# alexncoleman/WeaklySupervisedDL

Hardware: AMD Instinct MI355X
Metric: SegmentationModel train img/s at B=16 256x256 (higher is better)
Workload: dtype f32

## Files before the change

### weaklysuperviseddl_amd/csrc/conv_igemm.hip

```cpp
#include "common.h"

#include <type_traits>
#include <algorithm>
#include <cstdint>
#include <mutex>

typedef float f32x16 __attribute__((ext_vector_type(16)));

namespace {

constexpr int kThreads = 256;

struct ConvSrc {
    const float* x;
    const float* wt;
    const float* x_amax;
    int KH, KW, bh, ch, K, Cin;
    long long x_bs;
    unsigned x_bytes;
};

struct ConvP {
    const float* x;
    const float* wt;
    float* y;
    const float* scale;
    const float* shift;
    const float* res;
    int B, Cin, H, W, Cout, OH, OW, KH, KW;
    int ah, bh, ch, sh;
    int K;
    long long x_bs, y_bs, res_bs;
    int relu, accumulate;
    int P;
    unsigned x_bytes;
    int ksplit;
    float* slab;
    int ow0, own;
    int nb;
    int b_ow0[4], b_own[4], b_tile0[5];
    int grid_x;
    int xcd_py;
    int xcd_rowfast;
    int tile_img_major;
    const float* x_amax;
    float* y_amax;
    const uint8_t* acc_mask;
    const float* acc_base;
    int nsrc;
    ConvSrc src[3];
};

__device__ __forceinline__ float acc_prev(const ConvP& p, const float* ptr) {
    float o = *ptr;
    if (p.acc_mask) {
        const long long e = ptr - p.acc_base;
        if (!((p.acc_mask[e >> 3] >> (e & 7)) & 1)) o = 0.f;
    }
    return o;
}

template <int BM, int BN, int WM, bool ALIGNED>
__global__ __launch_bounds__(kThreads) void conv_igemm_kernel(ConvP p) {
    constexpr int BK = 16;
    constexpr int WN = 4 / WM;
    constexpr int MI = BM / WM / 32;
    constexpr int NI = BN / WN / 32;
    static_assert(MI >= 1 && NI >= 1 && MI * 32 * WM == BM && NI * 32 * WN == BN, "bad tile");
    constexpr int A_F4 = BK * BM / 4 / kThreads;
    constexpr int B_STEP = kThreads / BN;
    constexpr int B_PER = BK / B_STEP;

    __shared__ float As[2][BK * BM];
    __shared__ float Bs[2][BK * BN];
    __shared__ int vtaps[64];
    constexpr int kTab = ALIGNED ? 1 : 1024;
    __shared__ int ktab[kTab][2];

    const int tid = threadIdx.x;
    const int lane = tid & 63, wid = tid >> 6;
    const int wm = wid / WN, wn = wid % WN;
    const int m0 = blockIdx.y * BM;
    const int n0 = blockIdx.x * BN;
    const int OHOW = p.OH * p.OW;
    const int HW = p.H * p.W;
    const bool use_tab = !ALIGNED && p.K <= kTab;
    if (use_tab) {
        for (int k = tid; k < p.K; k += kThreads) {
            const int tp = k / p.Cin, ci = k - tp * p.Cin;
            const int ti = tp / p.KW, tj = tp - ti * p.KW;
            ktab[k][0] = ci * HW;
            ktab[k][1] = (int)(((unsigned)(ti * p.bh) << 16) | ((unsigned)(tj * p.bh) & 0xffffu));
        }
        __syncthreads();
    }

    const int pl = tid % BN, kr = tid / BN;
// ... 1103 lines not shown
            for (int pix = c0; pix < c0 + BK && pix < P && !any; ++pix) {
                const int r = pix % OHW, ih = (r / own) * stride + dh, iw = (ow0 + r % own) * stride + dw;
                any = ih >= 0 && ih < H && iw >= 0 && iw < W;
            }
            done += any;
            ++all;
        }
    }
    return all ? (double)done / (double)all : 1.0;
}

wsdl::Opt g_tile_threshold{400};
wsdl::Opt g_group_tps10{45};
constexpr int kNumCU = 256, kLdsPerCU = 160 * 1024;

template <int BM, int BN, int WM, int BK>
int launch_fast(const ConvP& p, hipStream_t s, dim3 grid) {
    grid.z = p.ksplit > 1 ? p.ksplit : 1;
    constexpr size_t static_lds = 2 * BK * (BM + BN) * sizeof(float) + 64 * sizeof(int);
    static std::once_flag once;
    std::call_once(once, [] {
        (void)hipFuncSetAttribute(reinterpret_cast<const void*>(&conv_igemm_fast_kernel<BM, BN, WM, BK>),
                                  hipFuncAttributeMaxDynamicSharedMemorySize, kLdsPerCU - (int)static_lds - 2048);
    });
    WSDL_TRACE("fp32_fast<%d,%d,%d> ks=%d nb=%d grid=%ux%ux%u", BM, BN, BK, p.ksplit, p.nb, grid.x, grid.y, grid.z);
    hipLaunchKernelGGL((conv_igemm_fast_kernel<BM, BN, WM, BK>), grid, dim3(kThreads), 0, s, p);
    WSDL_LAUNCH_CHECK();
    return WSDL_OK;
}

wsdl::Opt g_conv_split{1};
wsdl::Opt g_conv_arith{1};
bool split_eligible(int rows, int kc, int T) {
    return g_conv_split && kc % 16 == 0 && T <= 9 && split_layout_bytes(g_conv_arith, (long long)T * kc, rows) < (1ll << 31);
}

wsdl::Opt g_xcd_map{1};
int choose_xcd_py(const ConvP& p, int gx, int gy) {
    if (!g_xcd_map || p.ksplit > 1 || ((long long)gx * gy) % 8 != 0) return 0;
    const double wb = (g_conv_arith ? 4.0 : 6.0) * (double)p.K * p.Cout, xb = 4.0 * (double)p.B * p.Cin * p.H * p.W;
    int best = 0;
    double best_cost = 0.0;
    for (int py = 1; py <= 8; py *= 2) {
        const int px = 8 / py;
        if (gy % py || gx % px) continue;
        if (g_xcd_map > 10 && py != g_xcd_map - 10) continue;
        const double cost = wb * px + xb * py;
        if (!best || cost < best_cost) { best = py; best_cost = cost; }
    }
    if (g_xcd_map == 1 && (best <= 1 || best_cost > 0.9 * (wb * 8 + xb))) return 0;
    return best;
}

template <int BM, int BN, int WM, int BK>
int launch_split(const ConvP& p_in, hipStream_t s, dim3 grid) {
    ConvP p = p_in;
    grid.z = p.ksplit > 1 ? p.ksplit : 1;
    p.xcd_py = choose_xcd_py(p, grid.x, grid.y);
    p.tile_img_major = 0;
    constexpr bool MF = BK == 32;
    WSDL_TRACE("split<%d,%d,%d> ar=%d %s ks=%d xcd_py=%d nb=%d grid=%ux%ux%u", BM, BN, BK, (int)g_conv_arith,
               (MF && g_conv_arith) ? "mfma16x16x32" : "mfma32x32x16", p.ksplit, p.xcd_py, p.nb, grid.x, grid.y, grid.z);
    if (g_conv_arith == 2)
        hipLaunchKernelGGL((conv_igemm_split_kernel<BM, BN, WM, BK, kThreads, 2, MF>), grid, dim3(kThreads), 0, s, p);
    else if (g_conv_arith)
        hipLaunchKernelGGL((conv_igemm_split_kernel<BM, BN, WM, BK, kThreads, 1, MF>), grid, dim3(kThreads), 0, s, p);
    else
        hipLaunchKernelGGL((conv_igemm_split_kernel<BM, BN, WM, BK, kThreads, 0>), grid, dim3(kThreads), 0, s, p);
    WSDL_LAUNCH_CHECK();
    return WSDL_OK;
}

wsdl::Opt g_conv_il{1};
int launch_split_256x128(const ConvP& p_in, hipStream_t s) {
    ConvP p = p_in;
    dim3 grid(p.grid_x > 0 ? p.grid_x : wsdl::cdiv(p.P, 128), wsdl::cdiv(p.Cout, 256), p.ksplit > 1 ? p.ksplit : 1);
    p.xcd_py = choose_xcd_py(p, grid.x, grid.y);
    p.xcd_rowfast = 0;
    p.tile_img_major = 0;
    if (p.nsrc > 0 && grid.y % 2 == 0 && ((long long)grid.x * grid.y) % 8 == 0) {
        int py = 4;
        while (py > 1 && (grid.y % py || grid.x % (8 / py))) py /= 2;
        if (grid.y % py == 0 && grid.x % (8 / py) == 0) {
            p.xcd_py = py;
            p.xcd_rowfast = 1;
        }
    }
    WSDL_TRACE("split<256,128,16> ar=%d il=%d nsrc=%d ks=%d xcd_py=%d rowfast=%d imgmajor=%d nb=%d grid=%ux%ux%u", (int)g_conv_arith,
               (int)(g_conv_arith == 1 && g_conv_il), p.nsrc, p.ksplit, p.xcd_py, p.xcd_rowfast, p.tile_img_major, p.nb, grid.x, grid.y, grid.z);
    if (p.nsrc > 0) {
        if (g_conv_arith == 2) hipLaunchKernelGGL((conv_igemm_split_kernel<256, 128, 4, 16, 512, 2, false, true>), grid, dim3(512), 0, s, p);
        else if (g_conv_arith && g_conv_il)
            hipLaunchKernelGGL((conv_igemm_split_kernel<256, 128, 4, 16, 512, 1, false, true, true>), grid, dim3(512), 0, s, p);
        else if (g_conv_arith) hipLaunchKernelGGL((conv_igemm_split_kernel<256, 128, 4, 16, 512, 1, false, true>), grid, dim3(512), 0, s, p);
        else hipLaunchKernelGGL((conv_igemm_split_kernel<256, 128, 4, 16, 512, 0, false, true>), grid, dim3(512), 0, s, p);
        WSDL_LAUNCH_CHECK();
        return WSDL_OK;
    }
    if (g_conv_arith == 2) hipLaunchKernelGGL((conv_igemm_split_kernel<256, 128, 4, 16, 512, 2>), grid, dim3(512), 0, s, p);
    else if (g_conv_arith && g_conv_il)
        hipLaunchKernelGGL((conv_igemm_split_kernel<256, 128, 4, 16, 512, 1, false, false, true>), grid, dim3(512), 0, s, p);
    else if (g_conv_arith) hipLaunchKernelGGL((conv_igemm_split_kernel<256, 128, 4, 16, 512, 1>), grid, dim3(512), 0, s, p);
    else hipLaunchKernelGGL((conv_igemm_split_kernel<256, 128, 4, 16, 512, 0>), grid, dim3(512), 0, s, p);
    WSDL_LAUNCH_CHECK();
    return WSDL_OK;
}

template <int BM, int BN, int WM>
int launch_cfg(const ConvP& p, hipStream_t s, bool aligned, bool split) {
    dim3 grid(p.grid_x > 0 ? p.grid_x : wsdl::cdiv(p.P, BN), wsdl::cdiv(p.Cout, BM));
    constexpr bool kSmallTile = BM * BN <= 128 * 64;
    if (split) {
        if constexpr (kSmallTile) {
            if (p.Cin % 32 == 0) {
                return launch_split<BM, BN, WM, 32>(p, s, grid);
            }
        }
        return launch_split<BM, BN, WM, 16>(p, s, grid);
    } else if (aligned) {
        if constexpr (kSmallTile) {
            if (p.Cin % 32 == 0) {
                return launch_fast<BM, BN, WM, 32>(p, s, grid);
            }
        }
        return launch_fast<BM, BN, WM, 16>(p, s, grid);
    } else {
        WSDL_TRACE("fp32_generic<%d,%d> grid=%ux%u", BM, BN, grid.x, grid.y);
        hipLaunchKernelGGL((conv_igemm_kernel<BM, BN, WM, false>), grid, dim3(kThreads), 0, s, p);
    }
    WSDL_LAUNCH_CHECK();
    return WSDL_OK;
}

wsdl::Opt g_ksplit_target{512}, g_ksplit_max{8}, g_ksplit_min_chunks{4};
int igemm_ksplit(int P, int Cout, int Cin, int T, int dil) {
    if (Cin % 32 != 0 || Cout % 4 != 0 || Cout <= 64) return 1;
    const long long blocks = (long long)wsdl::cdiv(P, 64) * wsdl::cdiv(Cout, 128);
    const int nq = T * (Cin / 32);
    const long long b128 = (long long)wsdl::cdiv(P, 128) * wsdl::cdiv(Cout, 128);
    if (b128 >= 200 && b128 < g_tile_threshold && nq >= 64) return 2;
    if (blocks >= 160 || nq < 8) return 1;
    long long s = g_ksplit_target / blocks;
// ... 571 lines not shown
    WSDL_REQUIRE(ws_bytes >= wsdl_conv2d_fwd_group_workspace(n, k, dil, B, Cin, H, W, Cout) && (ws || ws_bytes == 0),
                 "conv2d_fwd_group: workspace too small");
    hipStream_t s = wsdl::as_stream(stream);
    ConvGroup grp{};
    grp.n = n;
    int order[4] = {0, 1, 2, 3};
    std::stable_sort(order, order + n, [&](int a, int b) {
        return group_max_taps(H, W, k[a], dil[a]) > group_max_taps(H, W, k[b], dil[b]); });
    unsigned char* wsp = static_cast<unsigned char*>(ws);
    int start = 0;
    double flops = 0.0, executed = 0.0, bytes = 4.0 * (double)B * Cin * H * W;
    const long long xbs = x_bs ? x_bs : (long long)Cin * H * W;
    for (int j = 0; j < n; ++j) {
        const int i = order[j];
        WSDL_REQUIRE(wt_fwd[i] && y[i], "conv2d_fwd_group: null problem %d", i);
        WSDL_REQUIRE((k[i] == 1 || k[i] == 3) && dil[i] >= 1, "conv2d_fwd_group: problem %d: 1x1 or 3x3, stride 1", i);
        WSDL_REQUIRE(split_eligible(Cout, Cin, k[i] * k[i]), "conv2d_fwd_group: problem %d is not on the split kernels", i);
        ConvP& p = grp.p[j];
        const int pad = dil[i] * (k[i] - 1) / 2;
        p.x = x; p.wt = static_cast<const float*>(wt_fwd[i]); p.y = y[i];
        p.B = B; p.Cin = Cin; p.H = H; p.W = W; p.Cout = Cout; p.OH = H; p.OW = W; p.KH = p.KW = k[i];
        p.ah = 1; p.bh = dil[i]; p.ch = -pad; p.sh = 1;
        p.K = k[i] * k[i] * Cin;
        p.x_bs = xbs;
        p.y_bs = (y_bs && y_bs[i]) ? y_bs[i] : (long long)Cout * H * W;
        p.res_bs = p.y_bs;
        WSDL_REQUIRE(p.x_bs >= (long long)Cin * H * W && p.y_bs >= (long long)Cout * H * W, "conv2d_fwd_group: batch stride smaller than an image");
        p.P = B * H * W;
        p.x_bytes = (unsigned)(((long long)(B - 1) * p.x_bs + (long long)Cin * H * W) * 4);
        p.x_amax = x_amax;
        p.ow0 = 0; p.own = W; p.nb = 1;
        Band bands[8];
        int nb = 1;
        bands[0] = Band{0, W};
        nb = column_bands(W, W, p.ah, p.bh, p.ch, p.sh, p.KW, bands);
        int tiles = 0;
        for (int b = 0; b < nb && nb > 1; ++b) {
            p.b_ow0[b] = bands[b].ow0;
            p.b_own[b] = bands[b].own;
            p.b_tile0[b] = tiles;
            tiles += wsdl::cdiv((long long)B * H * bands[b].own, 128);
        }
        p.nb = nb;
        p.b_tile0[nb > 1 ? nb : 0] = tiles;
        const int gx = nb > 1 ? tiles : wsdl::cdiv(p.P, 128), gy = Cout / 256;
        const int ks = group_ksplit(group_max_taps(H, W, k[i], dil[i]));
        p.ksplit = ks;
        if (ks > 1) {
            p.slab = reinterpret_cast<float*>(wsp);
            wsp += wsdl::align_up((size_t)ks * Cout * p.P * sizeof(float), 256);
        }
        p.xcd_py = (start % 8 == 0) ? choose_xcd_py(p, gx, gy) : 0;
        p.tile_img_major = k[i] > 1;
        grp.start[j] = start;
        grp.gx[j] = gx;
        grp.gy[j] = gy;
        start += gx * gy * ks;
        const double f = 2.0 * p.P * (double)Cout * p.K;
        flops += f;
        if (wsdl::prof_enabled()) {
            for (int b = 0; b < nb; ++b) {
                ConvP q = p;
                q.ow0 = bands[b].ow0; q.own = bands[b].own; q.P = B * H * q.own;
                executed += f * ((double)q.own / W) * igemm_executed_fraction(q, 128);
            }
        }
        bytes += 4.0 * ((double)p.K * Cout + (double)p.P * Cout);
    }
    grp.start[n] = start;
    {
        int ns = 0;
        bool same = true;
        for (int j = 0; j < n; ++j) {
            ns += grp.p[j].ksplit;
            same = same && grp.gx[j] * grp.gy[j] == grp.gx[0] * grp.gy[0];
        }
        if (same && ns <= 8 && (8 % ns == 0)) {
            grp.ns = ns;
            int s = 0;
            for (int j = 0; j < n; ++j)
                for (int z = 0; z < grp.p[j].ksplit; ++z) {
                    grp.s_prob[s] = j;
                    grp.s_slice[s] = z;
                    ++s;
                }
            for (int j = 0; j < n; ++j) grp.p[j].xcd_py = 0;
        }
    }
    {
        wsdl::ProfScope prof(WSDL_PROF_SPLIT_GROUP, s, flops, wsdl::prof_enabled() ? executed : flops, bytes);
        WSDL_TRACE("group split<256,128,16> ar=%d il=%d problems=%d streams=%d ks=%d/%d/%d/%d workgroups=%d", (int)g_conv_arith,
                   (int)(g_conv_arith == 1 && g_conv_il), n, grp.ns, grp.p[0].ksplit, n > 1 ? grp.p[1].ksplit : 0,
                   n > 2 ? grp.p[2].ksplit : 0, n > 3 ? grp.p[3].ksplit : 0, start);
        if (g_conv_arith == 2)
            hipLaunchKernelGGL((conv_igemm_split_group_kernel<256, 128, 4, 16, 512, 2>), dim3(start), dim3(512), 0, s, grp);
        else if (g_conv_arith && g_conv_il)
            hipLaunchKernelGGL((conv_igemm_split_group_kernel<256, 128, 4, 16, 512, 1, false, true>), dim3(start), dim3(512), 0, s, grp);
        else if (g_conv_arith)
            hipLaunchKernelGGL((conv_igemm_split_group_kernel<256, 128, 4, 16, 512, 1>), dim3(start), dim3(512), 0, s, grp);
        else
            hipLaunchKernelGGL((conv_igemm_split_group_kernel<256, 128, 4, 16, 512, 0>), dim3(start), dim3(512), 0, s, grp);
        WSDL_LAUNCH_CHECK();
    }
    for (int j = 0; j < n; ++j) {
        const ConvP& p = grp.p[j];
        if (p.ksplit <= 1) continue;
        const long long total = (long long)p.Cout * p.P;
        const bool vec4 = p.y_bs % 4 == 0 && (reinterpret_cast<uintptr_t>(p.y) & 15) == 0;
        if (vec4)
            hipLaunchKernelGGL(conv_splitk_reduce_vec4_kernel, dim3((int)std::min<long long>((total / 4 + 255) / 256, 8192)),
                               dim3(256), 0, s, p);
        else
            hipLaunchKernelGGL(conv_splitk_reduce_kernel, dim3((int)std::min<long long>((total + 255) / 256, 4096)),
                               dim3(256), 0, s, p);
        WSDL_LAUNCH_CHECK();
    }
    return WSDL_OK;
}

int wsdl_conv2d_dgrad_multi_ok(int n, int B, int Cin, int H, int W, int Cout) {
    if (n < 2 || n > 4 || !g_conv_split) return 0;
    if (Cin % 256 != 0 || Cout % 16 != 0) return 0;
    if ((long long)wsdl::cdiv((long long)B * H * W, 128) * (Cin / 256) < 256) return 0;
    if ((long long)wsdl::cdiv((long long)B * H * W, 128) * wsdl::cdiv(Cin, 128) < g_tile_threshold) return 0;
    if (igemm_ksplit(B * H * W, Cin, Cout, 9, 1) != 1) return 0;
    if (((long long)(B - 1) * Cout * H * W + (long long)Cout * H * W) * 4 > (1ll << 31) - 4) return 0;
    return 1;
}

int wsdl_conv2d_dgrad_multi(int n, const float* const* dy, const void* const* wt_dgrad, const float* const* dy_amax,
                            const int* k, const int* dil, const long long* dy_bs, float* dx, int B, int Cin, int H, int W,
                            int Cout, int accumulate, wsdl_stream_t stream) {
    WSDL_REQUIRE(dy && wt_dgrad && dy_amax && k && dil && dx, "conv2d_dgrad_multi: null pointer");
    WSDL_REQUIRE(wsdl_conv2d_dgrad_multi_ok(n, B, Cin, H, W, Cout), "conv2d_dgrad_multi: geometry not supported (see "
                 "wsdl_conv2d_dgrad_multi_ok): %d sources, B %d, %d -> %d channels, %d x %d", n, B, Cin, Cout, H, W);
    ConvP p{};
    double flops = 0.0;
    for (int i = 0; i < n; ++i) {
        WSDL_REQUIRE(dy[i] && wt_dgrad[i], "conv2d_dgrad_multi: null source %d", i);
        WSDL_REQUIRE((k[i] == 1 || k[i] == 3) && dil[i] >= 1, "conv2d_dgrad_multi: source %d: 1x1 or 3x3, stride 1", i);
        WSDL_REQUIRE(split_eligible(Cin, Cout, k[i] * k[i]), "conv2d_dgrad_multi: source %d is not on the split kernels", i);
        WSDL_REQUIRE(!g_conv_arith || dy_amax[i], "conv2d_dgrad_multi: source %d: the fp16x2 kernels need dy_amax", i);
        const int pad = dil[i] * (k[i] - 1) / 2;
        const long long bs = (dy_bs && dy_bs[i]) ? dy_bs[i] : (long long)Cout * H * W;
        WSDL_REQUIRE(bs >= (long long)Cout * H * W, "conv2d_dgrad_multi: batch stride smaller than an image");
        const unsigned xbytes = (unsigned)(((long long)(B - 1) * bs + (long long)Cout * H * W) * 4);
// ... 560 lines not shown
```

### weaklysuperviseddl_amd/csrc/conv_split.h

```cpp
#pragma once

typedef __bf16 bf16x8 __attribute__((ext_vector_type(8)));
typedef __bf16 bf16x2 __attribute__((ext_vector_type(2)));
typedef _Float16 half8 __attribute__((ext_vector_type(8)));
typedef float f32x4 __attribute__((ext_vector_type(4)));

__device__ __forceinline__ void split3(float x0, float x1, unsigned& h, unsigned& m, unsigned& l) {
    f32x2 v = {x0, x1};
    h = __builtin_bit_cast(unsigned, __builtin_convertvector(v, bf16x2));
    f32x2 r = {x0 - __builtin_bit_cast(float, h << 16), x1 - __builtin_bit_cast(float, h & 0xffff0000u)};
    m = __builtin_bit_cast(unsigned, __builtin_convertvector(r, bf16x2));
    f32x2 s = {r[0] - __builtin_bit_cast(float, m << 16), r[1] - __builtin_bit_cast(float, m & 0xffff0000u)};
    l = __builtin_bit_cast(unsigned, __builtin_convertvector(s, bf16x2));
}

__device__ __forceinline__ void split2hs(float x0, float x1, unsigned& h, unsigned& l) {
    f32x2 v = {x0, x1};
    const half2v hv = __builtin_convertvector(v, half2v);
    h = __builtin_bit_cast(unsigned, hv);
    f32x2 r = {(x0 - (float)hv[0]) * 2048.f, (x1 - (float)hv[1]) * 2048.f};
    l = __builtin_bit_cast(unsigned, __builtin_convertvector(r, half2v));
}

template <int AR> struct SplitArith;
// ... 58 lines not shown
    static_assert(B_PER == 4 || B_PER == 8 || B_PER == 16 || B_PER == 32, "B tile");
    constexpr unsigned kOOB = 0x80000000u;

    __shared__ __attribute__((aligned(16))) unsigned char As[2][BM * ROW];
    __shared__ __attribute__((aligned(16))) unsigned char Bs[2][BN * ROW];
    __shared__ int vtaps[64];

    const int tid = threadIdx.x;
    const int lane = tid & 63, wid = tid >> 6;
    const int wm = wid / WN, wn = wid % WN;
    int bx = bx_in, by = by_in;
    if (p.xcd_py > 0) {
        const int gx = grid_x;
        const int L = by * gx + bx;
        const int xcd = L & 7, idx = L >> 3;
        const int py = p.xcd_py, px = 8 / py;
        const int lx = gx / px, ly = grid_y / py;
        if (p.xcd_rowfast) {
            bx = (xcd / py) * lx + idx / ly;
            by = (xcd % py) * ly + idx % ly;
        } else {
            bx = (xcd / py) * lx + idx % lx;
            by = (xcd % py) * ly + idx / lx;
        }
    }
    const int m0 = by * BM;
    int w_ow0 = p.ow0, w_own = p.own, w_tile0 = 0;
    if (p.nb > 1) {
        w_ow0 = p.b_ow0[0];
        w_own = p.b_own[0];
#pragma unroll
        for (int i = 1; i < 4; ++i)
            if (i < p.nb && bx >= p.b_tile0[i]) {
                w_ow0 = p.b_ow0[i];
                w_own = p.b_own[i];
                w_tile0 = p.b_tile0[i];
            }
    }
    const int W_P = p.nb > 1 ? p.B * p.OH * w_own : p.P;
    int lt = bx - w_tile0;
    if (p.tile_img_major) {
        const int ohw = p.OH * w_own;
        const int tpi = ohw / BN;
        if (tpi > 1 && tpi * BN == ohw) lt = (lt % p.B) * tpi + lt / p.B;
    }
    const int n0 = lt * BN;
    const int OHOW = p.OH * p.OW;
    const int HW = p.H * p.W;

    const int pl = tid % BN;
    const int kr = tid / BN;
    const int pix = n0 + pl;
    const bool pix_ok = pix < W_P;
    int pb = 0, poh = 0, pow_ = 0;
    const int OHW = p.OH * w_own;
    if (pix_ok) {
        pb = pix / OHW;
        const int r = pix - pb * OHW;
        poh = r / w_own;
        pow_ = w_ow0 + (r - poh * w_own);
    }

    constexpr int TS = MF ? 16 : 32;
    constexpr int TMI = BM / WM / TS, TNI = BN / WN / TS;
    constexpr int RT = TS * TS / 64;
    using acc_t = std::conditional_t<MF, f32x4, f32x16>;
    acc_t acc[TMI][TNI];
    constexpr int LO = AR == 2 ? 1 : 0;
    acc_t acc_lo[LO ? TMI : 1][LO ? TNI : 1];
#pragma unroll
    for (int i = 0; i < TMI; ++i)
#pragma unroll
        for (int j = 0; j < TNI; ++j)
#pragma unroll
            for (int r = 0; r < RT; ++r) {
                acc[i][j][r] = 0.f;
                if constexpr (LO) acc_lo[i][j][r] = 0.f;
            }
    const int l31 = MF ? (lane & 15) : (lane & 31), lh = MF ? (lane >> 4) : (lane >> 5);
    auto acc_row = [&](int r) { return MF ? lh * 4 + r : (r & 3) + 8 * (r >> 2) + 4 * lh; };

    float out_scale = 1.f;
    int e_units = 0;
    const int n_src = MS ? p.nsrc + 1 : 1;
    for (int src = 0; src < n_src; ++src) {
#define WSDL_SRC(f) ((!MS || src == 0) ? p.f : src == 1 ? p.src[0].f : src == 2 ? p.src[1].f : p.src[2].f)
    const float* const s_x = WSDL_SRC(x);
    const float* const s_wt = WSDL_SRC(wt);
    const float* const s_amax = WSDL_SRC(x_amax);
    const int s_KH = WSDL_SRC(KH), s_KW = WSDL_SRC(KW), s_bh = WSDL_SRC(bh), s_ch = WSDL_SRC(ch);
    const int s_K = WSDL_SRC(K), s_Cin = WSDL_SRC(Cin);
    const long long s_x_bs = WSDL_SRC(x_bs);
    const unsigned s_x_bytes = WSDL_SRC(x_bytes);
#undef WSDL_SRC

    const int wbytes = (s_K / 16) * p.Cout * K16B;
    const __amdgpu_buffer_rsrc_t rx = __builtin_amdgcn_make_buffer_rsrc(const_cast<float*>(s_x), 0, (int)s_x_bytes, 0x00020000);
    const __amdgpu_buffer_rsrc_t rw = __builtin_amdgcn_make_buffer_rsrc(const_cast<float*>(s_wt), 0, wbytes, 0x00020000);
    float xs = 1.f;
    if constexpr (AR >= 1) {
        int ex, ew;
        xs = pow2_scale(*s_amax, ex);
        (void)pow2_scale(*reinterpret_cast<const float*>(reinterpret_cast<const unsigned char*>(s_wt) + wbytes), ew);
        out_scale = pow2(-(ex + ew));
        if constexpr (MS) {
            if (src > 0 && ex + ew != e_units) {
                const float f = pow2(ex + ew - e_units);
#pragma unroll
                for (int i = 0; i < TMI; ++i)
#pragma unroll
                    for (int j = 0; j < TNI; ++j)
#pragma unroll
                        for (int r = 0; r < RT; ++r) {
                            acc[i][j][r] *= f;
                            if constexpr (LO) acc_lo[i][j][r] *= f;
                        }
            }
            e_units = ex + ew;
        }
    }
    const unsigned img_off = (unsigned)((long long)pb * s_x_bs) + (unsigned)(kr * B_PER * HW);

    auto tap_src = [&](int t, int& sp) {
        const int ti = t / s_KW, tj = t - ti * s_KW;
        const int nh = poh * p.ah + ti * s_bh + s_ch;
        const int nw = pow_ * p.ah + tj * s_bh + s_ch;
        bool ok = pix_ok && nh >= 0 && nw >= 0;
        int ih = nh, iw = nw;
        if (p.sh != 1) {
            ih = nh / p.sh;
            iw = nw / p.sh;
            ok = ok && (ih * p.sh == nh) && (iw * p.sh == nw);
        }
        ok = ok && ih < p.H && iw < p.W;
        sp = ih * p.W + iw;
        return ok;
    };

    const int T = s_KH * s_KW;
    const int cpt = s_Cin / BK;
    int nv = 0;
    for (int t = 0; t < T; ++t) {
        int sp;
        const bool ok = tap_src(t, sp);
        if (__syncthreads_or(ok)) {
            if (tid == 0) vtaps[nv] = t;
            ++nv;
        }
    }
    const int nq_all = nv * cpt;
    const int q0 = p.ksplit > 1 ? (int)((long long)nq_all * bz / p.ksplit) : 0;
    const int q1 = p.ksplit > 1 ? (int)((long long)nq_all * (bz + 1) / p.ksplit) : nq_all;
    const int nq = q1 - q0;
    __syncthreads();

    constexpr bool kRowMajorA = UPR == 4 && (A_UPS % 64) == 0;
    unsigned voff_a[A_U], lds_a[A_U];
#pragma unroll
    for (int e = 0; e < A_U; ++e) {
        const int u = tid + e * NT;
        const int ks = u / A_UPS, v = u - ks * A_UPS;
        const int j = v & 63;
        const int row = kRowMajorA ? (v >> 6) * 16 + (j & 7) + 8 * (j >> 5) : v / UPR;
        const int part = kRowMajorA ? (j >> 3) & 3 : v - row * UPR;
        voff_a[e] = (m0 + row < p.Cout && (A_EXACT || u < KS * A_UPS))
                        ? (unsigned)(ks * p.Cout * K16B + ((m0 + row) * UPR + part) * 16) : kOOB;
        if constexpr (MF)
            lds_a[e] = (unsigned)(row * ROW + (((4 * (part >> 1) + 2 * ks + (part & 1)) ^ (row & 7)) << 4));
        else
            lds_a[e] = (unsigned)(row * ROW + ks * K16B + part * 16);
    }

    u32x4 ra[A_U];
    unsigned rb[B_PER];
    int ld_vi = q0 / cpt, ld_c = q0 - (q0 / cpt) * cpt, ld_tap = 0;
    unsigned voff_b = kOOB;
    auto set_tap = [&](int vi) {
        ld_tap = __builtin_amdgcn_readfirstlane(vtaps[vi]);
        int sp;
        const bool ok = tap_src(ld_tap, sp);
        voff_b = ok ? (img_off + (unsigned)sp) * 4u : kOOB;
    };
    if (nq > 0) set_tap(ld_vi);

    auto load_next = [&]() {
        if (ld_c == cpt) {
            ld_c = 0;
            ++ld_vi;
            set_tap(ld_vi);
        }
        const int c16 = (ld_tap * s_Cin + ld_c * BK) / 16;
        const unsigned soff_a = (unsigned)(c16 * p.Cout * K16B);
#pragma unroll
        for (int e = 0; e < A_U; ++e) ra[e] = __builtin_amdgcn_raw_buffer_load_b128(rw, voff_a[e], soff_a, 0);
        const unsigned soff_b = (unsigned)(ld_c * BK * HW) * 4u;
#pragma unroll
        for (int e = 0; e < B_PER; ++e)
            rb[e] = __builtin_amdgcn_raw_buffer_load_b32(rx, voff_b, soff_b + (unsigned)(e * HW) * 4u, 0);
        ++ld_c;
    };
    auto store_tiles = [&](int buf) {
#pragma unroll
        for (int e = 0; e < A_U; ++e)
            if (A_EXACT || tid + e * NT < KS * A_UPS) *reinterpret_cast<u32x4*>(&As[buf][lds_a[e]]) = ra[e];
        unsigned pc[NP][B_PER / 2];
#pragma unroll
        for (int e = 0; e < B_PER / 2; ++e) {
            const float x0 = __builtin_bit_cast(float, rb[2 * e]), x1 = __builtin_bit_cast(float, rb[2 * e + 1]);
            if constexpr (AR == 0)
                split3(x0, x1, pc[0][e], pc[1][e], pc[2][e]);
            else if constexpr (AR == 1)
                split2h(x0 * xs, x1 * xs, pc[0][e], pc[1][e]);
            else
                split2hs(x0 * xs, x1 * xs, pc[0][e], pc[1][e]);
        }
        unsigned char* rowp = &Bs[buf][pl * ROW];
        if constexpr (MF) {
            static_assert(!MF || B_PER == 8 || B_PER == 16 || B_PER == 32, "a thread's run is whole k-groups");
#pragma unroll
            for (int g = 0; g < B_PER / 8; ++g) {
                const int kg = kr * (B_PER / 8) + g;
#pragma unroll
                for (int c = 0; c < NP; ++c)
                    *reinterpret_cast<u32x4*>(rowp + (((4 * c + kg) ^ (pl & 7)) << 4)) =
                        u32x4{pc[c][4 * g], pc[c][4 * g + 1], pc[c][4 * g + 2], pc[c][4 * g + 3]};
            }
        } else if constexpr (B_PER == 4) {
            const int k = kr * 4, off = (k / 16) * K16B + (k % 16) * 2;
#pragma unroll
            for (int c = 0; c < NP; ++c) *reinterpret_cast<u32x2*>(rowp + off + c * 32) = u32x2{pc[c][0], pc[c][1]};
        } else {
#pragma unroll
            for (int g = 0; g < B_PER / 8; ++g) {
                const int k = kr * B_PER + g * 8, off = (k / 16) * K16B + (k % 16) * 2;
#pragma unroll
                for (int c = 0; c < NP; ++c)
                    *reinterpret_cast<u32x4*>(rowp + off + c * 32) =
                        u32x4{pc[c][4 * g], pc[c][4 * g + 1], pc[c][4 * g + 2], pc[c][4 * g + 3]};
            }
        }
    };

    if (nq > 0) {
        load_next();
        store_tiles(0);
        if (nq > 1) load_next();
    }
    __syncthreads();
    auto mfma_chunk = [&](int cur) {
        if constexpr (MF) {
            const unsigned char* Ab = As[cur] + (wm * (BM / WM) + l31) * ROW;
            const unsigned char* Bb = Bs[cur] + (wn * (BN / WN) + l31) * ROW;
            const unsigned f0 = (unsigned)((lh ^ (l31 & 7)) << 4), f1 = (unsigned)(((4 + lh) ^ (l31 & 7)) << 4);
            half8 a[TMI][2], b[TNI][2];
#pragma unroll
            for (int i = 0; i < TMI; ++i) {
                a[i][0] = *reinterpret_cast<const half8*>(Ab + i * 16 * ROW + f0);
                a[i][1] = *reinterpret_cast<const half8*>(Ab + i * 16 * ROW + f1);
            }
#pragma unroll
            for (int j = 0; j < TNI; ++j) {
                b[j][0] = *reinterpret_cast<const half8*>(Bb + j * 16 * ROW + f0);
                b[j][1] = *reinterpret_cast<const half8*>(Bb + j * 16 * ROW + f1);
            }
#pragma unroll
            for (int i = 0; i < TMI; ++i)
#pragma unroll
                for (int j = 0; j < TNI; ++j) {
                    if constexpr (LO) {
                        f32x4 c = acc_lo[i][j];
                        c = __builtin_amdgcn_mfma_f32_16x16x32_f16(a[i][1], b[j][0], c, 0, 0, 0);
                        c = __builtin_amdgcn_mfma_f32_16x16x32_f16(a[i][0], b[j][1], c, 0, 0, 0);
                        acc_lo[i][j] = c;
                        acc[i][j] = __builtin_amdgcn_mfma_f32_16x16x32_f16(a[i][0], b[j][0], acc[i][j], 0, 0, 0);
                    } else {
                        f32x4 c = acc[i][j];
                        c = __builtin_amdgcn_mfma_f32_16x16x32_f16(a[i][1], b[j][0], c, 0, 0, 0);
                        c = __builtin_amdgcn_mfma_f32_16x16x32_f16(a[i][0], b[j][1], c, 0, 0, 0);
                        c = __builtin_amdgcn_mfma_f32_16x16x32_f16(a[i][0], b[j][0], c, 0, 0, 0);
                        acc[i][j] = c;
                    }
                }
        } else {
            const unsigned char* Ab = As[cur] + (wm * (MI * 32) + l31) * ROW + lh * 16;
            const unsigned char* Bb = Bs[cur] + (wn * (NI * 32) + l31) * ROW + lh * 16;
#pragma unroll
            for (int ks = 0; ks < KS; ++ks) {
                frag a[MI][NP], b[NI][NP];
#pragma unroll
                for (int i = 0; i < MI; ++i)
#pragma unroll
                    for (int c = 0; c < NP; ++c)
                        a[i][c] = *reinterpret_cast<const frag*>(Ab + i * 32 * ROW + ks * K16B + c * 32);
#pragma unroll
                for (int j = 0; j < NI; ++j)
#pragma unroll
                    for (int c = 0; c < NP; ++c)
                        b[j][c] = *reinterpret_cast<const frag*>(Bb + j * 32 * ROW + ks * K16B + c * 32);
#pragma unroll
                for (int i = 0; i < MI; ++i)
#pragma unroll
                    for (int j = 0; j < NI; ++j) {
                        if constexpr (!MF && LO) {
                            acc_lo[i][j] = Ar::mma(a[i][1], b[j][0], acc_lo[i][j]);
                            acc_lo[i][j] = Ar::mma(a[i][0], b[j][1], acc_lo[i][j]);
                            acc[i][j] = Ar::mma(a[i][0], b[j][0], acc[i][j]);
                        } else if constexpr (!MF) {
                            acc[i][j] = split_products<AR>(a[i], b[j], acc[i][j]);
                        }
                    }
            }
        }
    };
    int q_start = 0;
    if constexpr (IL) {
        static_assert(!IL || (!MF && KS == 1 && AR == 1), "interleaved loop: 32x32x16 form, K chunk 16, fp16x2");
        unsigned il_soff_a = 0, il_soff_b = 0;
        auto advance = [&]() {
            if (ld_c == cpt) {
                ld_c = 0;
                ++ld_vi;
                set_tap(ld_vi);
            }
            il_soff_a = (unsigned)(((ld_tap * s_Cin + ld_c * BK) / 16) * p.Cout * K16B);
            il_soff_b = (unsigned)(ld_c * BK * HW) * 4u;
            ++ld_c;
        };
        const unsigned fra = (unsigned)((wm * (MI * 32) + l31) * ROW + lh * 16), frb = (unsigned)((wn * (NI * 32) + l31) * ROW + lh * 16);
        int q = 0;
        if (nq > 2) advance();
        for (; q + 2 < nq; ++q) {
            const int cur = q & 1;
            frag a[MI][NP], b[NI][NP];
#pragma unroll
            for (int i = 0; i < MI; ++i)
#pragma unroll
                for (int c = 0; c < NP; ++c) a[i][c] = *reinterpret_cast<const frag*>(&As[cur][fra + i * 32 * ROW + c * 32]);
#pragma unroll
            for (int j = 0; j < NI; ++j)
#pragma unroll
                for (int c = 0; c < NP; ++c) b[j][c] = *reinterpret_cast<const frag*>(&Bs[cur][frb + j * 32 * ROW + c * 32]);
            store_tiles(cur ^ 1);
#pragma unroll
            for (int e = 0; e < A_U; ++e) ra[e] = __builtin_amdgcn_raw_buffer_load_b128(rw, voff_a[e], il_soff_a, 0);
#pragma unroll
            for (int e = 0; e < B_PER; ++e)
                rb[e] = __builtin_amdgcn_raw_buffer_load_b32(rx, voff_b, il_soff_b + (unsigned)(e * HW) * 4u, 0);
#pragma unroll
            for (int i = 0; i < MI; ++i)
#pragma unroll
                for (int j = 0; j < NI; ++j) acc[i][j] = split_products<AR>(a[i], b[j], acc[i][j]);
            __builtin_amdgcn_sched_group_barrier(0x100, (MI + NI) * NP, 0);
            __builtin_amdgcn_sched_group_barrier(0x002, 4, 0);
#pragma unroll
            for (int k = 0; k < MI * NI * 3; ++k) {
                __builtin_amdgcn_sched_group_barrier(0x008, 1, 0);
                __builtin_amdgcn_sched_group_barrier(0x002, 2, 0);
                if (k < 4) __builtin_amdgcn_sched_group_barrier(0x200, 1, 0);
                else if (k < 4 + A_U + B_PER) __builtin_amdgcn_sched_group_barrier(0x020, 1, 0);
            }
            lds_barrier();
            if (q + 3 < nq) advance();
        }
        q_start = q;
    }
    for (int q = q_start; q < nq; ++q) {
        const int cur = q & 1;
        if (q + 1 < nq) {
            store_tiles(cur ^ 1);
        }
        if (q + 2 < nq) load_next();
        mfma_chunk(cur);
        lds_barrier();
    }
    }

    if (p.ksplit > 1) {
        float* sl = p.slab + (long long)bz * p.Cout * p.P;
#pragma unroll
        for (int j = 0; j < TNI; ++j) {
            const int opix = n0 + wn * (BN / WN) + j * TS + l31;
            if (opix >= W_P) continue;
            const int ob = opix / OHW;
            const int orr = opix - ob * OHW, ooh = orr / w_own;
            const int gpix = ob * OHOW + ooh * p.OW + w_ow0 + (orr - ooh * w_own);
#pragma unroll
            for (int i = 0; i < TMI; ++i)
#pragma unroll
                for (int r = 0; r < RT; ++r) {
                    const int co = m0 + wm * (BM / WM) + i * TS + acc_row(r);
                    float v = acc[i][j][r];
                    if constexpr (LO) v = fmaf(acc_lo[i][j][r], 0x1p-11f, v);
                    if (co < p.Cout) sl[(long long)co * p.P + gpix] = AR >= 1 ? v * out_scale : v;
                }
        }
        return;
    }
    float vmax = 0.f;
#pragma unroll
    for (int j = 0; j < TNI; ++j) {
        const int opix = n0 + wn * (BN / WN) + j * TS + l31;
        if (opix >= W_P) continue;
        const int ob = opix / OHW;
        const int orr = opix - ob * OHW, ooh = orr / w_own;
        const int orp = ooh * p.OW + w_ow0 + (orr - ooh * w_own);
        float* yb = p.y + (long long)ob * p.y_bs + orp;
        const float* rbp = p.res ? p.res + (long long)ob * p.res_bs + orp : nullptr;
#pragma unroll
        for (int i = 0; i < TMI; ++i) {
#pragma unroll
            for (int r = 0; r < RT; ++r) {
                const int co = m0 + wm * (BM / WM) + i * TS + acc_row(r);
                if (co >= p.Cout) continue;
                float v = acc[i][j][r];
                if constexpr (LO) v = fmaf(acc_lo[i][j][r], 0x1p-11f, v);
                if constexpr (AR >= 1) v *= out_scale;
                if (p.scale) v *= p.scale[co];
                if (p.shift) v += p.shift[co];
                const long long off = (long long)co * OHOW;
                if (rbp) v += rbp[off];
                if (p.accumulate) v += acc_prev(p, yb + off);
                if (p.relu) v = fmaxf(v, 0.f);
                yb[off] = v;
                vmax = fmaxf(vmax, fabsf(v));
            }
        }
    }
    if (p.y_amax) publish_amax(vmax, p.y_amax);
}

template <int BM, int BN, int WM, int BK, int NT = kThreads, int AR = 1, bool MF = false, bool MS = false, bool IL = false>
__global__ __launch_bounds__(NT, NT == kThreads ? 2 : 1) void conv_igemm_split_kernel(ConvP p) {
    conv_igemm_split_body<BM, BN, WM, BK, NT, AR, MF, MS, IL>(p, blockIdx.x, blockIdx.y, blockIdx.z, gridDim.x, gridDim.y);
}

struct ConvGroup {
    int n;
    int start[5];
    int gx[4], gy[4];
    int ns;
    int s_prob[8], s_slice[8];
    ConvP p[4];
};
template <int BM, int BN, int WM, int BK, int NT = kThreads, int AR = 1, bool MF = false, bool IL = false>
__global__ __launch_bounds__(NT, NT == kThreads ? 2 : 1) void conv_igemm_split_group_kernel(ConvGroup grp) {
    const int L = blockIdx.x;
    if (grp.ns > 0) {
        const int s = L % grp.ns, r = L / grp.ns;
        const int g = grp.s_prob[s], gx = grp.gx[g], gy = grp.gy[g];
        conv_igemm_split_body<BM, BN, WM, BK, NT, AR, MF, false, IL>(grp.p[g], r % gx, r / gx, grp.s_slice[s], gx, gy);
        return;
    }
    int g = 0;
#pragma unroll
    for (int i = 1; i < 4; ++i)
        if (i < grp.n && L >= grp.start[i]) g = i;
    const int local = L - grp.start[g], gx = grp.gx[g], gy = grp.gy[g];
    const int plane = gx * gy, bz = local / plane, r = local - bz * plane;
    conv_igemm_split_body<BM, BN, WM, BK, NT, AR, MF, false, IL>(grp.p[g], r % gx, r / gx, bz, gx, gy);
}

__global__ void amax_kernel(const float* __restrict__ x, long long per, long long x_bs, long long total,
                            float* __restrict__ out) {
    float m = 0.f;
    if (x_bs == per && (per & 3) == 0 && (reinterpret_cast<unsigned long long>(x) & 15) == 0) {
        const float4* x4 = reinterpret_cast<const float4*>(x);
        for (long long i = blockIdx.x * (long long)blockDim.x + threadIdx.x; i < total / 4; i += (long long)gridDim.x * blockDim.x) {
            const float4 v = x4[i];
            m = fmaxf(fmaxf(m, fmaxf(fabsf(v.x), fabsf(v.y))), fmaxf(fabsf(v.z), fabsf(v.w)));
        }
    } else {
        for (long long i = blockIdx.x * (long long)blockDim.x + threadIdx.x; i < total; i += (long long)gridDim.x * blockDim.x) {
            const long long b = i / per;
            m = fmaxf(m, fabsf(x[b * x_bs + (i - b * per)]));
        }
    }
    publish_amax(m, out);
}

__global__ void multi_amax_kernel(const float* const* __restrict__ ptrs, const long long* __restrict__ counts,
                                  float* __restrict__ out) {
    const float* x = ptrs[blockIdx.y];
    const long long n = counts[blockIdx.y];
    float m = 0.f;
    if ((n & 3) == 0 && (reinterpret_cast<unsigned long long>(x) & 15) == 0) {
// ... 867 lines not shown
```

Before: 906.6.

## Reorder conv implicit-GEMM K loop to iterate taps inside channel chunks

Result: no change. 908.4, median of 6 (+0.2%).

```diff
diff --git a/weaklysuperviseddl_amd/csrc/conv_igemm.hip b/weaklysuperviseddl_amd/csrc/conv_igemm.hip
--- a/weaklysuperviseddl_amd/csrc/conv_igemm.hip
+++ b/weaklysuperviseddl_amd/csrc/conv_igemm.hip
@@ -3,6 +3,7 @@
 #include <type_traits>
 #include <algorithm>
 #include <cstdint>
+#include <cstdlib>
 #include <mutex>
 
 typedef float f32x16 __attribute__((ext_vector_type(16)));
@@ -43,6 +44,7 @@
     int xcd_py;
     int xcd_rowfast;
     int tile_img_major;
+    int k_taps_inner;
     const float* x_amax;
     float* y_amax;
     const uint8_t* acc_mask;
@@ -1252,15 +1254,31 @@
     return best;
 }
 
+constexpr int kTapsInnerMinCin = 1024;
+int choose_k_taps_inner(const ConvP& p) {
+    if (p.ah != 1 || p.sh != 1) return 0;
+    if ((p.bh < 0 ? p.Cout : p.Cin) < kTapsInnerMinCin) return 0;
+    bool multi_tap = false;
+    for (int i = 0; i <= p.nsrc; ++i) {
+        const int taps = i ? p.src[i - 1].KH * p.src[i - 1].KW : p.KH * p.KW;
+        const long long bh = std::abs(i ? p.src[i - 1].bh : p.bh), ch = std::abs(i ? p.src[i - 1].ch : p.ch);
+        if (taps <= 1) continue;
+        if (taps > 9 || (2 * bh + ch) * (p.W + 1) >= (1ll << 17)) return 0;
+        multi_tap = true;
+    }
+    return multi_tap ? 1 : 0;
+}
+
 template <int BM, int BN, int WM, int BK>
 int launch_split(const ConvP& p_in, hipStream_t s, dim3 grid) {
     ConvP p = p_in;
     grid.z = p.ksplit > 1 ? p.ksplit : 1;
     p.xcd_py = choose_xcd_py(p, grid.x, grid.y);
     p.tile_img_major = 0;
+    p.k_taps_inner = choose_k_taps_inner(p);
     constexpr bool MF = BK == 32;
-    WSDL_TRACE("split<%d,%d,%d> ar=%d %s ks=%d xcd_py=%d nb=%d grid=%ux%ux%u", BM, BN, BK, (int)g_conv_arith,
-               (MF && g_conv_arith) ? "mfma16x16x32" : "mfma32x32x16", p.ksplit, p.xcd_py, p.nb, grid.x, grid.y, grid.z);
+    WSDL_TRACE("split<%d,%d,%d> ar=%d %s ks=%d xcd_py=%d korder=%d nb=%d grid=%ux%ux%u", BM, BN, BK, (int)g_conv_arith,
+               (MF && g_conv_arith) ? "mfma16x16x32" : "mfma32x32x16", p.ksplit, p.xcd_py, p.k_taps_inner, p.nb, grid.x, grid.y, grid.z);
     if (g_conv_arith == 2)
         hipLaunchKernelGGL((conv_igemm_split_kernel<BM, BN, WM, BK, kThreads, 2, MF>), grid, dim3(kThreads), 0, s, p);
     else if (g_conv_arith)
@@ -1278,6 +1296,7 @@
     p.xcd_py = choose_xcd_py(p, grid.x, grid.y);
     p.xcd_rowfast = 0;
     p.tile_img_major = 0;
+    p.k_taps_inner = choose_k_taps_inner(p);
     if (p.nsrc > 0 && grid.y % 2 == 0 && ((long long)grid.x * grid.y) % 8 == 0) {
         int py = 4;
         while (py > 1 && (grid.y % py || grid.x % (8 / py))) py /= 2;
@@ -1286,8 +1305,9 @@
             p.xcd_rowfast = 1;
         }
     }
-    WSDL_TRACE("split<256,128,16> ar=%d il=%d nsrc=%d ks=%d xcd_py=%d rowfast=%d imgmajor=%d nb=%d grid=%ux%ux%u", (int)g_conv_arith,
-               (int)(g_conv_arith == 1 && g_conv_il), p.nsrc, p.ksplit, p.xcd_py, p.xcd_rowfast, p.tile_img_major, p.nb, grid.x, grid.y, grid.z);
+    WSDL_TRACE("split<256,128,16> ar=%d il=%d nsrc=%d ks=%d xcd_py=%d rowfast=%d imgmajor=%d korder=%d nb=%d grid=%ux%ux%u", (int)g_conv_arith,
+               (int)(g_conv_arith == 1 && g_conv_il), p.nsrc, p.ksplit, p.xcd_py, p.xcd_rowfast, p.tile_img_major, p.k_taps_inner, p.nb,
+               grid.x, grid.y, grid.z);
     if (p.nsrc > 0) {
         if (g_conv_arith == 2) hipLaunchKernelGGL((conv_igemm_split_kernel<256, 128, 4, 16, 512, 2, false, true>), grid, dim3(512), 0, s, p);
         else if (g_conv_arith && g_conv_il)
@@ -1965,6 +1985,7 @@
         }
         p.xcd_py = (start % 8 == 0) ? choose_xcd_py(p, gx, gy) : 0;
         p.tile_img_major = k[i] > 1;
+        p.k_taps_inner = choose_k_taps_inner(p);
         grp.start[j] = start;
         grp.gx[j] = gx;
         grp.gy[j] = gy;
@@ -2002,9 +2023,10 @@
     }
     {
         wsdl::ProfScope prof(WSDL_PROF_SPLIT_GROUP, s, flops, wsdl::prof_enabled() ? executed : flops, bytes);
-        WSDL_TRACE("group split<256,128,16> ar=%d il=%d problems=%d streams=%d ks=%d/%d/%d/%d workgroups=%d", (int)g_conv_arith,
+        WSDL_TRACE("group split<256,128,16> ar=%d il=%d problems=%d streams=%d ks=%d/%d/%d/%d korder=%d/%d/%d/%d workgroups=%d", (int)g_conv_arith,
                    (int)(g_conv_arith == 1 && g_conv_il), n, grp.ns, grp.p[0].ksplit, n > 1 ? grp.p[1].ksplit : 0,
-                   n > 2 ? grp.p[2].ksplit : 0, n > 3 ? grp.p[3].ksplit : 0, start);
+                   n > 2 ? grp.p[2].ksplit : 0, n > 3 ? grp.p[3].ksplit : 0, grp.p[0].k_taps_inner, n > 1 ? grp.p[1].k_taps_inner : 0,
+                   n > 2 ? grp.p[2].k_taps_inner : 0, n > 3 ? grp.p[3].k_taps_inner : 0, start);
         if (g_conv_arith == 2)
             hipLaunchKernelGGL((conv_igemm_split_group_kernel<256, 128, 4, 16, 512, 2>), dim3(start), dim3(512), 0, s, grp);
         else if (g_conv_arith && g_conv_il)
diff --git a/weaklysuperviseddl_amd/csrc/conv_split.h b/weaklysuperviseddl_amd/csrc/conv_split.h
--- a/weaklysuperviseddl_amd/csrc/conv_split.h
+++ b/weaklysuperviseddl_amd/csrc/conv_split.h
@@ -134,14 +134,7 @@
     const int kr = tid / BN;
     const int pix = n0 + pl;
     const bool pix_ok = pix < W_P;
-    int pb = 0, poh = 0, pow_ = 0;
     const int OHW = p.OH * w_own;
-    if (pix_ok) {
-        pb = pix / OHW;
-        const int r = pix - pb * OHW;
-        poh = r / w_own;
-        pow_ = w_ow0 + (r - poh * w_own);
-    }
 
     constexpr int TS = MF ? 16 : 32;
     constexpr int TMI = BM / WM / TS, TNI = BN / WN / TS;
@@ -176,6 +169,13 @@
     const unsigned s_x_bytes = WSDL_SRC(x_bytes);
 #undef WSDL_SRC
 
+    int pb = 0, poh = 0, pow_ = 0;
+    if (pix_ok) {
+        pb = pix / OHW;
+        const int r = pix - pb * OHW;
+        poh = r / w_own;
+        pow_ = w_ow0 + (r - poh * w_own);
+    }
     const int wbytes = (s_K / 16) * p.Cout * K16B;
     const __amdgpu_buffer_rsrc_t rx = __builtin_amdgcn_make_buffer_rsrc(const_cast<float*>(s_x), 0, (int)s_x_bytes, 0x00020000);
     const __amdgpu_buffer_rsrc_t rw = __builtin_amdgcn_make_buffer_rsrc(const_cast<float*>(s_wt), 0, wbytes, 0x00020000);
@@ -203,10 +203,10 @@
     }
     const unsigned img_off = (unsigned)((long long)pb * s_x_bs) + (unsigned)(kr * B_PER * HW);
 
-    auto tap_src = [&](int t, int& sp) {
+    auto tap_src = [&](int t, int oh, int ow, int& sp) {
         const int ti = t / s_KW, tj = t - ti * s_KW;
-        const int nh = poh * p.ah + ti * s_bh + s_ch;
-        const int nw = pow_ * p.ah + tj * s_bh + s_ch;
+        const int nh = oh * p.ah + ti * s_bh + s_ch;
+        const int nw = ow * p.ah + tj * s_bh + s_ch;
         bool ok = pix_ok && nh >= 0 && nw >= 0;
         int ih = nh, iw = nw;
         if (p.sh != 1) {
@@ -222,14 +222,21 @@
     const int T = s_KH * s_KW;
     const int cpt = s_Cin / BK;
     int nv = 0;
+    unsigned tap_word = 0;
     for (int t = 0; t < T; ++t) {
         int sp;
-        const bool ok = tap_src(t, sp);
+        const bool ok = tap_src(t, poh, pow_, sp);
         if (__syncthreads_or(ok)) {
             if (tid == 0) vtaps[nv] = t;
+            if (p.k_taps_inner) {
+                const int ti = t / s_KW, tj = t - ti * s_KW;
+                if (ok) tap_word |= 1u << nv;
+                if (lane == nv) tap_word |= (unsigned)(((ti * s_bh + s_ch) * p.W + (tj * s_bh + s_ch)) * 8192 + (t << 9));
+            }
             ++nv;
         }
     }
+    const bool kti = p.k_taps_inner && nv > 1;
     const int nq_all = nv * cpt;
     const int q0 = p.ksplit > 1 ? (int)((long long)nq_all * bz / p.ksplit) : 0;
     const int q1 = p.ksplit > 1 ? (int)((long long)nq_all * (bz + 1) / p.ksplit) : nq_all;
@@ -256,31 +263,25 @@
     u32x4 ra[A_U];
     unsigned rb[B_PER];
     int ld_vi = q0 / cpt, ld_c = q0 - (q0 / cpt) * cpt, ld_tap = 0;
+    if (kti) {
+        ld_c = q0 / nv;
+        ld_vi = q0 - ld_c * nv;
+    }
     unsigned voff_b = kOOB;
+    unsigned b_base = img_off;
+    int b_r0 = poh, b_r1 = pow_;
+    if (kti) {
+        b_base = img_off + (unsigned)(poh * p.W + pow_);
+        b_r0 = (int)tap_word;
+        b_r1 = 0;
+    }
     auto set_tap = [&](int vi) {
         ld_tap = __builtin_amdgcn_readfirstlane(vtaps[vi]);
         int sp;
-        const bool ok = tap_src(ld_tap, sp);
-        voff_b = ok ? (img_off + (unsigned)sp) * 4u : kOOB;
-    };
-    if (nq > 0) set_tap(ld_vi);
-
-    auto load_next = [&]() {
-        if (ld_c == cpt) {
-            ld_c = 0;
-            ++ld_vi;
-            set_tap(ld_vi);
-        }
-        const int c16 = (ld_tap * s_Cin + ld_c * BK) / 16;
-        const unsigned soff_a = (unsigned)(c16 * p.Cout * K16B);
-#pragma unroll
-        for (int e = 0; e < A_U; ++e) ra[e] = __builtin_amdgcn_raw_buffer_load_b128(rw, voff_a[e], soff_a, 0);
-        const unsigned soff_b = (unsigned)(ld_c * BK * HW) * 4u;
-#pragma unroll
-        for (int e = 0; e < B_PER; ++e)
-            rb[e] = __builtin_amdgcn_raw_buffer_load_b32(rx, voff_b, soff_b + (unsigned)(e * HW) * 4u, 0);
-        ++ld_c;
-    };
+        const bool ok = tap_src(ld_tap, b_r0, b_r1, sp);
+        voff_b = ok ? (b_base + (unsigned)sp) * 4u : kOOB;
+    };
+    if (nq > 0 && !kti) set_tap(ld_vi);
     auto store_tiles = [&](int buf) {
 #pragma unroll
         for (int e = 0; e < A_U; ++e)
@@ -323,12 +324,6 @@
         }
     };
 
-    if (nq > 0) {
-        load_next();
-        store_tiles(0);
-        if (nq > 1) load_next();
-    }
-    __syncthreads();
     auto mfma_chunk = [&](int cur) {
         if constexpr (MF) {
             const unsigned char* Ab = As[cur] + (wm * (BM / WM) + l31) * ROW;
@@ -394,19 +389,54 @@
             }
         }
     };
+    auto run_chunks = [&](auto kti_tag) {
+    const bool KTI = kti_tag;
+    auto next_chunk = [&]() {
+        if (KTI) {
+            if (ld_vi == nv) {
+                ld_vi = 0;
+                ++ld_c;
+            }
+            const int ent = __builtin_amdgcn_readlane(b_r0, ld_vi);
+            ld_tap = (ent >> 9) & 15;
+            voff_b = (((unsigned)b_r0 >> ld_vi) & 1u) ? (b_base + (unsigned)(ent >> 13)) * 4u : kOOB;
+            ++ld_vi;
+            return ld_c;
+        } else {
+            if (ld_c == cpt) {
+                ld_c = 0;
+                ++ld_vi;
+                set_tap(ld_vi);
+            }
+            return ld_c++;
+        }
+    };
+
+    auto load_next = [&]() {
+        const int c = next_chunk();
+        const int c16 = (ld_tap * s_Cin + c * BK) / 16;
+        const unsigned soff_a = (unsigned)(c16 * p.Cout * K16B);
+#pragma unroll
+        for (int e = 0; e < A_U; ++e) ra[e] = __builtin_amdgcn_raw_buffer_load_b128(rw, voff_a[e], soff_a, 0);
+        const unsigned soff_b = (unsigned)(c * BK * HW) * 4u;
+#pragma unroll
+        for (int e = 0; e < B_PER; ++e)
+            rb[e] = __builtin_amdgcn_raw_buffer_load_b32(rx, voff_b, soff_b + (unsigned)(e * HW) * 4u, 0);
+    };
+    if (nq > 0) {
+        load_next();
+        store_tiles(0);
+        if (nq > 1) load_next();
+    }
+    __syncthreads();
     int q_start = 0;
     if constexpr (IL) {
         static_assert(!IL || (!MF && KS == 1 && AR == 1), "interleaved loop: 32x32x16 form, K chunk 16, fp16x2");
         unsigned il_soff_a = 0, il_soff_b = 0;
         auto advance = [&]() {
-            if (ld_c == cpt) {
-                ld_c = 0;
-                ++ld_vi;
-                set_tap(ld_vi);
-            }
-            il_soff_a = (unsigned)(((ld_tap * s_Cin + ld_c * BK) / 16) * p.Cout * K16B);
-            il_soff_b = (unsigned)(ld_c * BK * HW) * 4u;
-            ++ld_c;
+            const int c = next_chunk();
+            il_soff_a = (unsigned)(((ld_tap * s_Cin + c * BK) / 16) * p.Cout * K16B);
+            il_soff_b = (unsigned)(c * BK * HW) * 4u;
         };
         const unsigned fra = (unsigned)((wm * (MI * 32) + l31) * ROW + lh * 16), frb = (unsigned)((wn * (NI * 32) + l31) * ROW + lh * 16);
         int q = 0;
@@ -455,6 +485,10 @@
         mfma_chunk(cur);
         lds_barrier();
     }
+    };
+    if constexpr (MS) run_chunks(kti);
+    else if (kti) run_chunks(std::true_type{});
+    else run_chunks(std::false_type{});
     }
 
     if (p.ksplit > 1) {
@@ -512,7 +546,7 @@
 }
 
 template <int BM, int BN, int WM, int BK, int NT = kThreads, int AR = 1, bool MF = false, bool MS = false, bool IL = false>
-__global__ __launch_bounds__(NT, NT == kThreads ? 2 : 1) void conv_igemm_split_kernel(ConvP p) {
+__global__ __launch_bounds__(NT, (IL && !MS) ? 4 : NT == kThreads ? 2 : 1) void conv_igemm_split_kernel(ConvP p) {
     conv_igemm_split_body<BM, BN, WM, BK, NT, AR, MF, MS, IL>(p, blockIdx.x, blockIdx.y, blockIdx.z, gridDim.x, gridDim.y);
 }
 
```
